# alibaba-damo-academy/Inferix

Hardware: AMD Instinct MI355X
Metric: latent_frames_per_sec (higher is better)
Workload: dtype bf16; 1 GPU; Self-Forcing 480p bf16 (Wan2.1-T2V-1.3B causal DiT, 30 layers), block_size=3, 21 latent frames = 7 blocks x (4 denoise + 1 context) generator forwards, KV prefix 4680..32760 keys in the KV manager's cache (identity page map; page-table form: `streaming_steady`); `value` counts the generator calls (SURVEY 8d), the per-block VAE decode of config 2 is measured beside it under --full (`per_block_decod; batch=1, parallelism=single, layers=30, pair_forwards=True, pair_mode=streams

## Files before the change

### inferix_amd/csrc/ifx_common.h

```cpp
#pragma once
#include <hip/hip_runtime.h>
#include <stdint.h>
#include <stdio.h>

#include "../../include/inferix_hip.h"

namespace ifx {

constexpr int kWave = 64;

typedef __attribute__((ext_vector_type(8))) __bf16 bf16x8;
typedef __attribute__((ext_vector_type(4))) __bf16 bf16x4;
typedef __attribute__((ext_vector_type(8))) unsigned short u16x8;
typedef __attribute__((ext_vector_type(4))) unsigned short u16x4;
typedef __attribute__((ext_vector_type(4))) short s16x4;
typedef __attribute__((ext_vector_type(4))) float f32x4;
typedef __attribute__((ext_vector_type(16))) float f32x16;
typedef __attribute__((ext_vector_type(4))) unsigned int u32x4;
typedef __attribute__((ext_vector_type(2))) unsigned int u32x2;

__device__ __forceinline__ float bf2f(unsigned short u) {
  return __builtin_bit_cast(float, (unsigned int)u << 16);
}
__device__ __forceinline__ unsigned short f2bf(float f) {
// ... 7 lines not shown
  float p = 0.17087277f;
  p = fmaf(p, t, -0.82215223f);
  p = fmaf(p, t, 1.48851587f);
  p = fmaf(p, t, -1.13520398f);
  p = fmaf(p, t, 0.27886807f);
  p = fmaf(p, t, -0.18628806f);
  p = fmaf(p, t, 0.09678418f);
  p = fmaf(p, t, 0.37409196f);
  p = fmaf(p, t, 1.00002368f);
  p = fmaf(p, t, -1.26551223f);
  const float arg = fmaf(-z, z, p);
  const float a = arg * 1.4426950408889634f;
  float r = fmaf(arg, 1.4426950408889634f, -a);
  r = fmaf(arg, 1.9259629911266175e-8f, r);
  const float ex = __builtin_amdgcn_exp2f(a) * fmaf(r, 0.6931471805599453f, 1.0f);
  const float erfc_z = t * ex;
  const float e = x >= 0.f ? 1.0f - erfc_z : erfc_z - 1.0f;
  return 0.5f * x * (1.0f + e);
}

__device__ __forceinline__ float gelu_tanh_fast(float x) {
  constexpr float c1 = -2.0f * 0.7978845608028654f * 1.4426950408889634f, c2 = c1 * 0.044715f;
  const float a = __builtin_fmaf(x * x, c2, c1) * x;
  return x * __builtin_amdgcn_rcpf(1.0f + __builtin_amdgcn_exp2f(a));
}

struct RowDivisor {
  float s, r;
  __device__ __forceinline__ explicit RowDivisor(float scale)
      : s(__builtin_bit_cast(float, __builtin_amdgcn_readfirstlane(__builtin_bit_cast(int, scale)))), r(__builtin_amdgcn_rcpf(s)) {}
  __device__ __forceinline__ bool fast() const { return s > 8.67361738e-19f && s < 1.15292150e18f; }
  template <bool FAST>
  __device__ __forceinline__ float div(float x) const {
    if (FAST) {
      const float q0 = x * r;
      const float e = __builtin_fmaf(-q0, s, x);
      return __builtin_fmaf(e, r, q0);
    }
    return x / s;
  }
};

template <int CTRL, int ROW_MASK>
__device__ __forceinline__ float dpp_or(float old, float v) {
  return __builtin_bit_cast(float, __builtin_amdgcn_update_dpp(__builtin_bit_cast(int, old), __builtin_bit_cast(int, v), CTRL, ROW_MASK, 0xf, false));
}
__device__ __forceinline__ float wave_sum(float v) {
  v += dpp_or<0xB1, 0xf>(0.f, v);
  v += dpp_or<0x4E, 0xf>(0.f, v);
  v += dpp_or<0x141, 0xf>(0.f, v);
  v += dpp_or<0x140, 0xf>(0.f, v);
  v += dpp_or<0x142, 0xa>(0.f, v);
  v += dpp_or<0x143, 0xc>(0.f, v);
  return __builtin_bit_cast(float, __builtin_amdgcn_readlane(__builtin_bit_cast(int, v), 63));
}
__device__ __forceinline__ float wave_max(float v) {
  v = fmaxf(v, dpp_or<0xB1, 0xf>(v, v));
  v = fmaxf(v, dpp_or<0x4E, 0xf>(v, v));
  v = fmaxf(v, dpp_or<0x141, 0xf>(v, v));
  v = fmaxf(v, dpp_or<0x140, 0xf>(v, v));
  v = fmaxf(v, dpp_or<0x142, 0xa>(v, v));
  v = fmaxf(v, dpp_or<0x143, 0xc>(v, v));
  return __builtin_bit_cast(float, __builtin_amdgcn_readlane(__builtin_bit_cast(int, v), 63));
}

struct KvAddr {
  const int32_t* pt;
  int32_t ps;
  int32_t seg_split, seg_delta;
  __device__ __forceinline__ int slot(int t) const {
    if (pt == nullptr) return (seg_split > 0 && t >= seg_split) ? t + seg_delta : t;
    int pg = t / ps;
    return pt[pg] * ps + (t - pg * ps);
  }
};

void set_error(const char* fmt, ...);
int check_launch(const char* what);
int gemm_variant();
int gemm_small_split();
unsigned* device_error_word();
long long spin_timeout_ticks();
int spin_fault();
int conv_variant();
unsigned* attn_debug_counter();
int attn_variant();

}

#define IFX_REQUIRE(cond, ...)            \
  do {                                    \
    if (!(cond)) {                        \
      ifx::set_error(__VA_ARGS__);        \
      return IFX_EINVAL;                  \
    }                                     \
  } while (0)
```

### inferix_amd/csrc/ifx_core.hip

```cpp
#include <stdarg.h>
#include <stdlib.h>
#include <string.h>

#include "ifx_common.h"

namespace ifx {
static thread_local char g_err[512] = "";

void set_error(const char* fmt, ...) {
  va_list ap;
  va_start(ap, fmt);
  vsnprintf(g_err, sizeof(g_err), fmt, ap);
  va_end(ap);
}

static int g_gemm_variant = -1, g_attn_variant = -1, g_conv_variant = -1, g_spin_timeout_ms = -1, g_spin_fault = 0;
static thread_local int g_gemm_small_split = -1;
static int opt_or_env(int& slot, const char* env, int dflt = 0) {
  if (slot < 0) {
    const char* e = getenv(env);
    slot = e ? atoi(e) : dflt;
  }
  return slot;
}
int gemm_variant() { return opt_or_env(g_gemm_variant, "IFX_GEMM_VARIANT"); }
int attn_variant() { return opt_or_env(g_attn_variant, "IFX_ATTN_VARIANT"); }
int conv_variant() { return opt_or_env(g_conv_variant, "IFX_CONV_VARIANT"); }
static unsigned* g_attn_dbg = nullptr;
static bool g_attn_dbg_on = false;
unsigned* attn_debug_counter() { return g_attn_dbg_on ? g_attn_dbg : nullptr; }
int gemm_small_split() { return opt_or_env(g_gemm_small_split, "IFX_GEMM_SMALL_SPLIT"); }

static unsigned* g_dev_err = nullptr;
unsigned* device_error_word() {
  if (g_dev_err == nullptr) {
    void* p = nullptr;
    if (hipHostMalloc(&p, 64, hipHostMallocMapped | hipHostMallocPortable) == hipSuccess && p != nullptr) {
      memset(p, 0, 64);
      g_dev_err = (unsigned*)p;
    }
  }
  return g_dev_err;
}
long long spin_timeout_ticks() { return (long long)max(1, opt_or_env(g_spin_timeout_ms, "IFX_SPIN_TIMEOUT_MS", 2000)) * 100000LL; }
int spin_fault() { return g_spin_fault; }
static thread_local char g_err_dev[640] = "";

int check_launch(const char* what) {
  hipError_t e = hipGetLastError();
  if (e != hipSuccess) {
    set_error("%s: launch failed: %s", what, hipGetErrorString(e));
    return IFX_ELAUNCH;
  }
  return IFX_OK;
}
}

extern "C" int ifx_version(void) { return (0 << 16) | (IFX_ABI_MINOR << 8) | 0; }
extern "C" int32_t ifx_device_error(int32_t clear) {
  unsigned* w = ifx::g_dev_err;
  if (w == nullptr) return 0;
  const unsigned v = __atomic_load_n(w, __ATOMIC_ACQUIRE);
  if (v != 0 && clear) __atomic_store_n(w, 0u, __ATOMIC_RELEASE);
  return (int32_t)v;
}
extern "C" const char* ifx_last_error(void) {
  const unsigned v = (unsigned)ifx_device_error(1);
  if (v == 0) return ifx::g_err;
  const unsigned kind = v >> 24, detail = v & 0xffffffu;
  snprintf(ifx::g_err_dev, sizeof(ifx::g_err_dev),
           "device: a kernel gave up a wait (%s, flag %u) after the spin budget — the producing workgroup was not resident or did not "
           "finish; the results of that launch are invalid%s%s",
           kind == 1 ? "split-K / stream-K consumer of ifx_gemm_bf16_ws / ifx_gemm_q8_ws" : "unknown waiter", detail,
           ifx::g_err[0] ? "; last host error: " : "", ifx::g_err);
  return ifx::g_err_dev;
}
extern "C" const char* ifx_arch(void) { return "gfx950"; }
extern "C" int ifx_set_option(const char* key, int32_t value) {
  if (key && !strcmp(key, "gemm_variant") && value >= 0 && value <= 29) { ifx::g_gemm_variant = value; return IFX_OK; }
  if (key && !strcmp(key, "gemm_small_split") && (value == 0 || value == 1)) { ifx::g_gemm_small_split = value; return IFX_OK; }
  if (key && !strcmp(key, "attn_variant") && value >= 0 && value <= 7) { ifx::g_attn_variant = value; return IFX_OK; }
  if (key && !strcmp(key, "conv_variant") && value >= 0 && value <= 1) { ifx::g_conv_variant = value; return IFX_OK; }
  if (key && !strcmp(key, "attn_debug_counters") && (value == 0 || value == 1)) {
    if (value == 1) {
      if (ifx::g_attn_dbg == nullptr && hipMalloc((void**)&ifx::g_attn_dbg, 64) != hipSuccess) {
        ifx::g_attn_dbg = nullptr;
        ifx::set_error("ifx_set_option: attn_debug_counters: hipMalloc failed");
        return IFX_ELAUNCH;
      }
      (void)hipDeviceSynchronize();
      (void)hipMemset(ifx::g_attn_dbg, 0, 64);
    }
    ifx::g_attn_dbg_on = value == 1;
    return IFX_OK;
  }
  if (key && !strcmp(key, "spin_timeout_ms") && value >= 1 && value <= 600000) { ifx::g_spin_timeout_ms = value; return IFX_OK; }
  if (key && !strcmp(key, "spin_fault") && (value == 0 || value == 1)) { ifx::g_spin_fault = value; return IFX_OK; }
  ifx::set_error("ifx_set_option: unknown key or value out of range: %s = %d", key ? key : "(null)", (int)value);
  return IFX_EINVAL;
}
extern "C" int ifx_get_option(const char* key, int32_t* value) {
  if (key == nullptr || value == nullptr) { ifx::set_error("ifx_get_option: null argument"); return IFX_EINVAL; }
  if (!strcmp(key, "gemm_variant")) { *value = ifx::gemm_variant(); return IFX_OK; }
  if (!strcmp(key, "gemm_small_split")) { *value = ifx::gemm_small_split(); return IFX_OK; }
  if (!strcmp(key, "attn_variant")) { *value = ifx::attn_variant(); return IFX_OK; }
  if (!strcmp(key, "conv_variant")) { *value = ifx::conv_variant(); return IFX_OK; }
  if (!strcmp(key, "attn_debug_counters")) { *value = ifx::g_attn_dbg_on ? 1 : 0; return IFX_OK; }
  if (!strcmp(key, "attn_rescale_count")) {
    unsigned v = 0;
    if (ifx::g_attn_dbg != nullptr) {
      (void)hipDeviceSynchronize();
      (void)hipMemcpy(&v, ifx::g_attn_dbg, sizeof(v), hipMemcpyDeviceToHost);
    }
    *value = (int32_t)(v & 0x7fffffffu);
    return IFX_OK;
  }
  if (!strcmp(key, "spin_timeout_ms")) { *value = (int32_t)(ifx::spin_timeout_ticks() / 100000LL); return IFX_OK; }
  if (!strcmp(key, "spin_fault")) { *value = ifx::spin_fault(); return IFX_OK; }
  ifx::set_error("ifx_get_option: unknown key: %s", key);
  return IFX_EINVAL;
}
```

### inferix_amd/csrc/ifx_gemm_pp.hip

```cpp
#include <stdlib.h>

#include <type_traits>

#include "ifx_common.h"

#ifndef IFX_PP_TRACE
#define IFX_PP_TRACE 0
#endif
#ifndef IFX_PP_LAB
#define IFX_PP_LAB IFX_PP_TRACE
#endif


namespace ifx {

struct EpiArgsP {
  const unsigned short* bias;
  const unsigned short* residual;
  int ld_res;
  const unsigned short* mod;
  int mod_slots, gate_slot, rows_per_group;
  const float* sa = nullptr;
  const float* sw = nullptr;
  const float* qdiv = nullptr;
  int q_via_bf16 = 0;
  unsigned short* y2 = nullptr;
  int ldy2 = 0, split_col = 0;
};

namespace gpp {
constexpr int BN = 256, BK = 64;
constexpr int SLOT = 16384, STAGE = 4 * SLOT, SCRATCH = 2 * STAGE;
constexpr int LDS_BYTES = SCRATCH + 32768;
constexpr int X_UP = 0, W_LO = SLOT, W_HI = 2 * SLOT, X_DN = 3 * SLOT;
typedef int v4i __attribute__((ext_vector_type(4)));
typedef int v8i __attribute__((ext_vector_type(8)));
typedef int v16i __attribute__((ext_vector_type(16)));
typedef __attribute__((address_space(3))) void* lds_ptr_t;

__device__ __forceinline__ void dma16(v4i rsrc, unsigned lds, int voff, int soff) {
  asm volatile("s_mov_b32 m0, %0\n\ts_nop 0\n\tbuffer_load_dwordx4 %1, %2, %3 offen lds"
               :
               : "s"(lds), "v"(voff), "s"(rsrc), "s"(soff)
               : "memory");
}
__device__ __forceinline__ v4i make_rsrc(const void* base, unsigned num_bytes) {
  const unsigned long long a = (unsigned long long)base;
  v4i r;
  r[0] = (int)(unsigned)a;
  r[1] = (int)((unsigned)(a >> 32) & 0xffffu);
  r[2] = (int)num_bytes;
  r[3] = 0x00020000;
  return r;
}
template <int N>
__device__ __forceinline__ void wait_vm() {
  asm volatile("s_waitcnt vmcnt(%0)" ::"n"(N) : "memory");
}
__device__ __forceinline__ void wait_lds() { __builtin_amdgcn_s_waitcnt(0xC07F); }

struct Cursor {
  int i, kt, g, rot, k0, len;
  int kb;
  unsigned stg;
  v4i rs;
};
}

template <int EPI, int TJ, int KS, int Q8 = 0>
__global__ __launch_bounds__(512, 2) void gemm_pp_kernel(const unsigned short* __restrict__ x, int ldx,
                                                         const unsigned short* __restrict__ w, unsigned short* __restrict__ y,
                                                         int ldy, int M, int N, int K, int tiles_m, int total, int per_xcd,
                                                         int wg_per_xcd, EpiArgsP ea, unsigned long long* __restrict__ trace, int dbg,
                                                         float* __restrict__ ws_part, unsigned* __restrict__ ws_flag,
                                                         unsigned* __restrict__ err_word, long long spin_ticks) {
  using namespace gpp;
  dbg = IFX_PP_LAB ? dbg : (dbg & 32);
  constexpr int BM = 64 * TJ;
  constexpr int GM = 4;
  constexpr bool RES = EPI == IFX_EPI_RESIDUAL || EPI == IFX_EPI_GATE_RES;
  extern __shared__ __attribute__((aligned(16))) unsigned char smem[];
  const int tid = threadIdx.x, lane = tid & 63;
  const int wave = __builtin_amdgcn_readfirstlane(tid >> 6);
  const int grp = wave >> 2, w4 = wave & 3;
  constexpr int ES = Q8 ? 1 : 2;
  const unsigned char* const xb = reinterpret_cast<const unsigned char*>(x);
  const unsigned char* const wb = reinterpret_cast<const unsigned char*>(w);
  constexpr bool SK = KS == 0;
  constexpr int KSD = KS > 0 ? KS : 1;
  const int S = K * ES / 128;
  const int KT = S / KSD;
  const int tiles_n = total / KSD / tiles_m;

  const int xcd = blockIdx.x & 7, slot_i = blockIdx.x >> 3;
  const int id_first = xcd * per_xcd + slot_i;
  const int id_end = min(xcd * per_xcd + per_xcd, total);
  if (!SK && id_first >= id_end) return;
  const int sk_P = (int)gridDim.x, sk_p = xcd * (sk_P >> 3) + slot_i;
  auto sk_start = [&](int q) __attribute__((always_inline)) { return (int)((long)q * total * S / sk_P); };
  const int sk_u0 = SK ? sk_start(sk_p) : 0, sk_u1 = SK ? sk_start(sk_p + 1) : 0;
  const int sk_t0 = SK ? sk_u0 / S : 0;
  const int n_my = SK ? (sk_u1 - 1) / S - sk_t0 + 1 : (id_end - id_first + wg_per_xcd - 1) / wg_per_xcd;
  const int G = SK ? sk_u1 - sk_u0 : n_my * KT;
  auto item_split = [&](int i) __attribute__((always_inline)) { return KS > 1 ? (id_first + i * wg_per_xcd) % KSD : 0; };
  auto item_tile = [&](int i) __attribute__((always_inline)) { return SK ? sk_t0 + i : (id_first + i * wg_per_xcd) / KSD; };
  auto item_k0 = [&](int i) __attribute__((always_inline)) { return SK ? (i == 0 ? sk_u0 - sk_t0 * S : 0) : item_split(i) * KT; };
  auto item_len = [&](int i) __attribute__((always_inline)) {
    return SK ? min(S, sk_u1 - (sk_t0 + i) * S) - (i == 0 ? sk_u0 - sk_t0 * S : 0) : KT;
  };
  auto item_dumps = [&](int i) __attribute__((always_inline)) { return SK ? (i == 0 && sk_u0 > sk_t0 * S) : (KS > 1 && item_split(i) >= 1); };
  auto item_parts = [&](int i) __attribute__((always_inline)) {
    if (!SK) return KS > 1 ? KS - 1 : 0;
    const int t_end = (sk_t0 + i + 1) * S;
    int n = 0;
    while (sk_p + 1 + n < sk_P && sk_start(sk_p + 1 + n) < t_end) ++n;
    return sk_u1 < t_end ? n : 0;
  };
  auto tile_base = [&](int i, int& m_base, int& n_base) __attribute__((always_inline)) {
    const int t_id = item_tile(i);
    const int grp_sz = GM * tiles_n;
    const int first_m = (t_id / grp_sz) * GM;
    const int gm = min(GM, tiles_m - first_m);
    const int rem = t_id % grp_sz;
    m_base = (first_m + rem % gm) * BM;
    n_base = (rem / gm) * BN;
  };

  const int r8 = lane >> 3, pc = lane & 7;
  const int prow = w4 * 8 + r8;
  const int ld_op = grp == 0 ? K : ldx;
  const int voff = prow * ld_op * ES + ((pc ^ ((prow >> 1) & 7)) << 4);
  const unsigned lds_piece0 = (unsigned)(unsigned long long)(lds_ptr_t)smem + w4 * 1024;
  auto cur_desc = [&](Cursor& c) __attribute__((always_inline)) {
    int mb, nb;
    tile_base(c.i, mb, nb);
    if (dbg & 1) mb = nb = 0;
    c.rot = (!SK && (dbg & 4)) ? ((nb / BN) * 3) % KT : 0;
    c.k0 = item_k0(c.i);
    c.len = item_len(c.i);
    c.kb = c.k0 * 128;
    if (grp == 0) c.rs = make_rsrc(wb + (size_t)nb * K * ES, (unsigned)min(((long)N - nb) * (long)K * ES, 0xffffffffL));
    else c.rs = make_rsrc(xb + (size_t)mb * ldx * ES, (unsigned)min(((long)M - mb - 1) * (long)ldx * ES + (long)K * ES, 0xffffffffL));
  };
  auto cur_init = [&](Cursor& c) __attribute__((always_inline)) {
    c.i = 0, c.kt = 0, c.g = 0, c.stg = 0;
    cur_desc(c);
  };
  auto cur_next = [&](Cursor& c) __attribute__((always_inline)) {
    ++c.g;
    c.stg ^= STAGE;
    c.kb += 128;
    if (++c.kt == c.len) {
      c.kt = 0;
      if (++c.i < n_my) cur_desc(c);
    }
  };
  auto issue = [&](const Cursor& c, int slot, int row0, int pieces) __attribute__((always_inline)) {
    const int kk = c.kt + c.rot;
    const int kb = IFX_PP_LAB ? ((!SK && kk >= KT ? kk - KT : kk) + c.k0) * 128 : c.kb;
    const unsigned p = lds_piece0 + c.stg + slot;
    if ((dbg & 8) && c.g >= 2) return;
#pragma unroll
    for (int q = 0; q < 4; ++q)
      if (q < pieces) dma16(c.rs, p + q * 4096, voff, kb + (row0 + q * 32) * ld_op * ES);
  };
  Cursor ca, cb;
  cur_init(ca);
  cur_init(cb);

  constexpr bool MF16 = Q8 == 0;
  const int l31 = lane & 31, hi = lane >> 5, l15 = lane & 15, q4 = lane >> 4;
  int lane_ks[4];
#pragma unroll
  for (int ks = 0; ks < 4; ++ks)
    lane_ks[ks] = MF16 ? l15 * 128 + ((((4 * ks + q4) & 7) ^ ((l15 >> 1) & 7)) << 4)
                       : l31 * 128 + (((2 * ks + hi) ^ ((l31 >> 1) & 7)) << 4);
  const int w_frag_off = (w4 >> 1) * SLOT + (w4 & 1) * 8192 + W_LO;
  const int x_frag_off = grp == 0 ? X_UP : X_DN;
  bf16x8 fx[4][TJ], fw[4][2], fx16[2 * TJ][2];
  int rg = 0;
  auto read_frags = [&]() __attribute__((always_inline)) {
    const unsigned char* st = smem + (rg & 1) * STAGE;
    if constexpr (MF16) {
#pragma unroll
      for (int kk = 0; kk < 2; ++kk) {
#pragma unroll
        for (int c = 0; c < 4; ++c) fw[c][kk] = *reinterpret_cast<const bf16x8*>(st + w_frag_off + lane_ks[kk] + c * 2048);
#pragma unroll
        for (int t = 0; t < 2 * TJ; ++t) fx16[t][kk] = *reinterpret_cast<const bf16x8*>(st + x_frag_off + lane_ks[kk] + t * 2048);
      }
    } else {
#pragma unroll
      for (int ks = 0; ks < 4; ++ks) {
#pragma unroll
        for (int i = 0; i < 2; ++i) fw[ks][i] = *reinterpret_cast<const bf16x8*>(st + w_frag_off + lane_ks[ks] + i * 4096);
#pragma unroll
        for (int j = 0; j < TJ; ++j) fx[ks][j] = *reinterpret_cast<const bf16x8*>(st + x_frag_off + lane_ks[ks] + j * 4096);
      }
    }
    ++rg;
  };

  f32x16 acc[2][TJ];
  f32x4 acc16[4][2 * TJ];
  auto quad = [&](int i, int j, int g) __attribute__((always_inline)) {
    if constexpr (MF16) return acc16[g][2 * j + i];
    else return f32x4{acc[i][j][4 * g], acc[i][j][4 * g + 1], acc[i][j][4 * g + 2], acc[i][j][4 * g + 3]};
  };
  auto mfma16 = [&](bool first) __attribute__((always_inline)) {
    const f32x4 z = {0.f, 0.f, 0.f, 0.f};
#pragma unroll
    for (int kk = 0; kk < 2; ++kk)
#pragma unroll
      for (int c = 0; c < 4; ++c)
#pragma unroll
        for (int t = 0; t < 2 * TJ; ++t)
          acc16[c][t] = __builtin_amdgcn_mfma_f32_16x16x32_bf16(fw[c][kk], fx16[t][kk], first && kk == 0 ? z : acc16[c][t], 0, 0, 0);
  };
  auto q8_mfma = [&](int kk, int i, int j, const f32x16 c) __attribute__((always_inline)) {
    const v8i a = __builtin_shufflevector(__builtin_bit_cast(v4i, fw[2 * kk][i]), __builtin_bit_cast(v4i, fw[2 * kk + 1][i]), 0, 1, 2, 3, 4, 5, 6, 7);
    const v8i b = __builtin_shufflevector(__builtin_bit_cast(v4i, fx[2 * kk][j]), __builtin_bit_cast(v4i, fx[2 * kk + 1][j]), 0, 1, 2, 3, 4, 5, 6, 7);
    return __builtin_amdgcn_mfma_scale_f32_32x32x64_f8f6f4(a, b, c, 0, 0, 0, 0x7f7f7f7f, 0, 0x7f7f7f7f);
  };
  auto i8_mfma = [&](int ks, int i, int j, const f32x16 c) __attribute__((always_inline)) {
    return __builtin_bit_cast(f32x16, __builtin_amdgcn_mfma_i32_32x32x32_i8(__builtin_bit_cast(v4i, fw[ks][i]), __builtin_bit_cast(v4i, fx[ks][j]),
                                                                            __builtin_bit_cast(v16i, c), 0, 0, 0));
  };
  auto mfma_first = [&]() __attribute__((always_inline)) {
    const f32x16 z = {0.f, 0.f, 0.f, 0.f, 0.f, 0.f, 0.f, 0.f, 0.f, 0.f, 0.f, 0.f, 0.f, 0.f, 0.f, 0.f};
    if constexpr (Q8 == 2) {
#pragma unroll
      for (int ks = 0; ks < 4; ++ks)
#pragma unroll
        for (int i = 0; i < 2; ++i)
#pragma unroll
          for (int j = 0; j < TJ; ++j) acc[i][j] = i8_mfma(ks, i, j, ks == 0 ? z : acc[i][j]);
      return;
    }
    if constexpr (Q8 == 1) {
#pragma unroll
      for (int i = 0; i < 2; ++i)
#pragma unroll
        for (int j = 0; j < TJ; ++j) acc[i][j] = q8_mfma(0, i, j, z);
#pragma unroll
      for (int i = 0; i < 2; ++i)
#pragma unroll
        for (int j = 0; j < TJ; ++j) acc[i][j] = q8_mfma(1, i, j, acc[i][j]);
      return;
    }
    mfma16(true);
  };
  auto mfma_next = [&]() __attribute__((always_inline)) {
    if constexpr (Q8 == 2) {
#pragma unroll
      for (int ks = 0; ks < 4; ++ks)
#pragma unroll
        for (int i = 0; i < 2; ++i)
#pragma unroll
          for (int j = 0; j < TJ; ++j) acc[i][j] = i8_mfma(ks, i, j, acc[i][j]);
      return;
    }
    if constexpr (Q8 == 1) {
#pragma unroll
      for (int kk = 0; kk < 2; ++kk)
#pragma unroll
        for (int i = 0; i < 2; ++i)
#pragma unroll
          for (int j = 0; j < TJ; ++j) acc[i][j] = q8_mfma(kk, i, j, acc[i][j]);
      return;
    }
    mfma16(false);
  };
// ... 219 lines not shown
      }
      wait_lds();
#pragma unroll
      for (int p = 0; p < 4; ++p) {
        const int mrow = p * 8 + rr;
        const int m = e_m0 + j * 32 + mrow;
        const u16x8 vv = *reinterpret_cast<const u16x8*>(rd + p * 1024 + ((cc ^ (mrow & 7)) << 4));
        if constexpr (RES) asm volatile("" : "+v"(e_res[j & 1][p]));
        if constexpr (EPI == IFX_EPI_GATE_RES) {
          if (j == 0 && p == 0) asm volatile("" : "+v"(e_gate[0]), "+v"(e_gate[1]));
        }
        u16x8 o;
        if constexpr (EPI == IFX_EPI_BIAS) {
          o = vv;
        } else if constexpr (EPI == IFX_EPI_GELU_TANH) {
          if (ea.gate_slot) {
#pragma unroll
            for (int e = 0; e < 8; ++e) o[e] = f2bf(gelu_erf_f(bf2f(vv[e])));
          } else {
#pragma unroll
            for (int e = 0; e < 8; ++e) o[e] = f2bf(gelu_tanh_fast(bf2f(vv[e])));
          }
        } else {
          const u16x8 rv = __builtin_bit_cast(u16x8, e_res[j & 1][p]);
          if constexpr (EPI == IFX_EPI_RESIDUAL) {
#pragma unroll
            for (int e = 0; e < 8; ++e) o[e] = f2bf(bf2f(rv[e]) + bf2f(vv[e]));
          } else {
            const u16x8 gv = __builtin_bit_cast(u16x8, m >= e_split ? e_gate[1] : e_gate[0]);
#pragma unroll
            for (int e = 0; e < 8; ++e) o[e] = f2bf(bf2f(rv[e]) + rbf(bf2f(vv[e]) * bf2f(gv[e])));
          }
        }
        if constexpr (Q8 && EPI == IFX_EPI_GELU_TANH) {
          if (ea.qdiv != nullptr) {
            unsigned wq[2];
#pragma unroll
            for (int h = 0; h < 2; ++h) {
              float t[4];
#pragma unroll
              for (int e = 0; e < 4; ++e) {
                const float q = fminf(fmaxf(bf2f(o[4 * h + e]) / e_qd[h][e], -448.0f), 448.0f);
                t[e] = ea.q_via_bf16 ? rbf(q) : q;
              }
              unsigned pk = __builtin_amdgcn_cvt_pk_fp8_f32(t[0], t[1], 0u, false);
              wq[h] = __builtin_amdgcn_cvt_pk_fp8_f32(t[2], t[3], pk, true);
            }
            if (m < M && n_ok)
              *reinterpret_cast<u32x2*>(reinterpret_cast<unsigned char*>(y) + (size_t)(e_m0 + rr + j * 32 + p * 8) * ldy + e_n0 + cc * 8) =
                  u32x2{wq[0], wq[1]};
            continue;
          }
        }
        if (m < M && n_ok) *reinterpret_cast<u16x8*>(yrow + (size_t)(j * 32 + p * 8) * ldo) = o;
      }
    }
  };

#if IFX_PP_TRACE
  unsigned long long seg[6] = {0, 0, 0, 0, 0, 0};
  unsigned long long t_last = __builtin_readcyclecounter();
  int seg_i = 0;
#define PP_STAMP()                                                 \
  do {                                                             \
    const unsigned long long t_now = __builtin_readcyclecounter(); \
    seg[seg_i] += t_now - t_last;                                  \
    t_last = t_now;                                                \
    seg_i = seg_i == 5 ? 0 : seg_i + 1;                            \
  } while (0)
#else
#define PP_STAMP() \
  do {             \
  } while (0)
#endif
#ifndef IFX_PP_STAGGER
#define IFX_PP_STAGGER 0
#endif
  auto roles = [&](auto stagger_tag) __attribute__((always_inline)) {
  constexpr bool reads_first = decltype(stagger_tag)::value;

  int kt = 0, it = 0;
  int klen = item_len(0);
  if (grp == 0) {
    issue(ca, W_LO, 0, 4), issue(ca, W_HI, 128, 4), cur_next(ca);
    wait_vm<0>();
    __builtin_amdgcn_s_barrier();
    for (int g = 0; g < G; ++g) {
      PP_STAMP();
      const bool epi = g > 0 && kt == 0;
      const bool issued = ca.g < G;
      const bool early_reads = reads_first && !epi;
      if (epi && KS != 1 && item_dumps(it - 1)) {
        if (issued) issue(ca, W_LO, 0, 4), issue(ca, W_HI, 128, 4), cur_next(ca);
        PP_STAMP();
        dump_partial(it - 1);
        wait_vm<0>();
        flag_pending = flag_of(it - 1) + 1;
        PP_STAMP();
        read_frags();
      } else if (epi) {
        if (KS != 1) consumer_sync(it - 1);
        epilogue(it - 1, [&]() __attribute__((always_inline)) {
          if (issued) issue(ca, W_LO, 0, 4), issue(ca, W_HI, 128, 4), cur_next(ca);
          PP_STAMP();
        });
        PP_STAMP();
        read_frags();
      } else if (early_reads) {
        read_frags();
        if (issued) issue(ca, W_LO, 0, 4), issue(ca, W_HI, 128, 4), cur_next(ca);
        PP_STAMP();
        PP_STAMP();
      } else {
        if (issued) issue(ca, W_LO, 0, 4), issue(ca, W_HI, 128, 4), cur_next(ca);
        PP_STAMP();
        PP_STAMP();
        read_frags();
      }
      wait_lds();
      __builtin_amdgcn_sched_barrier(0);
      PP_STAMP();
      __builtin_amdgcn_s_barrier();
      __builtin_amdgcn_sched_barrier(0);
      PP_STAMP();
      if (KS != 1 && flag_pending) {
        if (wave == 0 && !(dbg & 32)) __hip_atomic_store(ws_flag + flag_pending - 1, 1u, __ATOMIC_RELAXED, __HIP_MEMORY_SCOPE_AGENT);
        flag_pending = 0;
      }
      if (!(dbg & 2)) {
        if (kt == 0) mfma_first();
        else mfma_next();
      }
      if (++kt == klen) kt = 0, ++it, klen = it < n_my ? item_len(it) : 0;
      wait_vm<0>();
      __builtin_amdgcn_sched_barrier(0);
      PP_STAMP();
      __builtin_amdgcn_s_barrier();
      __builtin_amdgcn_sched_barrier(0);
    }
    if (KS != 1 && item_dumps(it - 1)) {
      dump_partial(it - 1);
      wait_vm<0>();
      flag_pending = flag_of(it - 1) + 1;
    } else {
      if (KS != 1) consumer_sync(it - 1);
      epilogue(it - 1, [&]() __attribute__((always_inline)) {});
    }
    if (KS != 1) {
      __builtin_amdgcn_s_barrier();
      if (flag_pending && wave == 0 && !(dbg & 32)) __hip_atomic_store(ws_flag + flag_pending - 1, 1u, __ATOMIC_RELAXED, __HIP_MEMORY_SCOPE_AGENT);
    }
  } else {
    issue(cb, X_UP, 0, TJ), cur_next(cb);
    issue(ca, X_DN, 32 * TJ, TJ), cur_next(ca);
    if (cb.g < G) issue(cb, X_UP, 0, TJ), cur_next(cb);
    if (G > 1) wait_vm<2 * TJ>();
    else wait_vm<TJ>();
    __builtin_amdgcn_s_barrier();
    if (G > 1) wait_vm<TJ>();
    else wait_vm<0>();
    __builtin_amdgcn_s_barrier();
    for (int g = 0; g < G; ++g) {
      PP_STAMP();
      const bool lower = ca.g < G, upper = cb.g < G;
      if (reads_first) {
        read_frags();
        if (lower) issue(ca, X_DN, 32 * TJ, TJ), cur_next(ca);
        if (upper) issue(cb, X_UP, 0, TJ), cur_next(cb);
        PP_STAMP();
        PP_STAMP();
      } else {
        if (lower) issue(ca, X_DN, 32 * TJ, TJ), cur_next(ca);
        if (upper) issue(cb, X_UP, 0, TJ), cur_next(cb);
        PP_STAMP();
        PP_STAMP();
        read_frags();
      }
      wait_lds();
      if (upper) wait_vm<2 * TJ>();
      else if (lower) wait_vm<TJ>();
      else wait_vm<0>();
      __builtin_amdgcn_sched_barrier(0);
      PP_STAMP();
      __builtin_amdgcn_s_barrier();
      __builtin_amdgcn_sched_barrier(0);
      PP_STAMP();
      if (!(dbg & 2)) {
        if (kt == 0) mfma_first();
        else mfma_next();
      }
      if (++kt == klen) kt = 0, ++it, klen = it < n_my ? item_len(it) : 0;
      if (upper) wait_vm<TJ>();
      else wait_vm<0>();
      __builtin_amdgcn_sched_barrier(0);
      PP_STAMP();
      if (kt == 0) {
        if (KS != 1 && item_dumps(it - 1)) {
          dump_partial(it - 1);
          wait_vm<0>();
        } else {
          if (KS != 1) consumer_sync(it - 1);
          epilogue(it - 1, [&]() __attribute__((always_inline)) {});
        }
      }
      if (g + 1 < G || KS != 1) {
        __builtin_amdgcn_s_barrier();
        __builtin_amdgcn_sched_barrier(0);
      }
    }
  }
  };
  if (IFX_PP_STAGGER && (w4 & 1)) roles(std::true_type{});
  else roles(std::false_type{});
#if IFX_PP_TRACE
  if (trace != nullptr && blockIdx.x == 0 && lane == 0 && (wave & 3) == 0) {
#pragma unroll
    for (int k = 0; k < 6; ++k) trace[grp * 8 + k] = seg[k];
    trace[grp * 8 + 6] = (unsigned long long)G;
  }
#endif
}

bool gemm_pp_split(int N, int K) {
  static int min_k = -1;
  if (min_k < 0) {
    const char* e = getenv("IFX_PP_SPLIT_MIN_K");
    min_k = e ? atoi(e) : 4096;
  }
  return K >= min_k && N <= 2048 && (K / 64) % 2 == 0;
}
size_t gemm_pp_stream_k_workspace_bytes() { return 4096 + (size_t)256 * 128 * 256 * 4; }
size_t gemm_pp_workspace_bytes(int M, int N, int K) {
  if (!gemm_pp_split(N, K)) return 0;
  const size_t tn = (size_t)(N + 255) / 256;
  const size_t t4 = (size_t)((M + 255) / 256) * tn, t3 = (size_t)((M + 191) / 192) * tn;
  if (t4 > 1024) return 0;
  const size_t b4 = t4 * 256 * 256 * 4, b3 = t3 <= 1024 ? t3 * 192 * 256 * 4 : 0;
  return 4096 + (b4 > b3 ? b4 : b3);
}

size_t gemm_pp_small_workspace_bytes(int M, int N, int ks) {
  if (ks <= 1) return 0;
  const size_t tiles = (size_t)((M + 127) / 128) * ((N + 255) / 256);
  return 4096 + tiles * (size_t)(ks - 1) * 128 * 256 * 4;
}

int launch_gemm_pp(const unsigned short* x, int ldx, const unsigned short* w, unsigned short* y, int ldy, int M, int N, int K,
                   int mode, const unsigned short* bias, const unsigned short* residual, int ld_res, const unsigned short* mod,
                   int mod_slots, int gate_slot, int rows_per_group, hipStream_t s, int tj, void* workspace, const float* q8_sa,
                   const float* q8_sw, const float* q8_qdiv, int q8_via_bf16, int stream_k, int q8_int8, int force_ks,
                   unsigned short* y2, int ldy2, int split_col) {
  using namespace gpp;
  const bool q8 = q8_sa != nullptr;
  EpiArgsP ea{bias, residual, ld_res, mod, mod_slots, gate_slot, rows_per_group, q8_sa, q8_sw, q8_qdiv, q8_via_bf16, y2, ldy2, split_col};
  if (y2 != nullptr && (q8 || split_col <= 0 || split_col % BN != 0 || split_col >= N || ldy2 % 8 != 0 || ((uintptr_t)y2 & 15))) {
    set_error("ifx_gemm_bf16: the second destination needs bf16 operands, 0 < split_col < N a multiple of %d, ldy2 %% 8 == 0 and a 16-byte aligned y2", BN);
    return IFX_EINVAL;
  }
  if (q8 && (K % 128 != 0 || ldx % 16 != 0 || ((uintptr_t)q8_sw & 15) || ((uintptr_t)q8_qdiv & 15))) {
    set_error("ifx_gemm_q8: the ping-pong tile needs K %% 128 == 0, ldx %% 16 == 0 and 16-byte aligned scale vectors (K = %d, ldx = %d)", K, ldx);
    return IFX_EINVAL;
  }
  if (N % 64 != 0 || K % 64 != 0) {
    set_error("ifx_gemm_bf16: the ping-pong tile needs N and K to be multiples of 64 (N = %d, K = %d)", N, K);
    return IFX_EINVAL;
  }
  if (mode == IFX_EPI_GATE_RES && rows_per_group < 32 * tj) {
    set_error("ifx_gemm_bf16: the ping-pong tile needs gate groups of at least %d rows (rows_per_group = %d)", 32 * tj, rows_per_group);
    return IFX_EINVAL;
  }
  const bool res = mode == IFX_EPI_RESIDUAL || mode == IFX_EPI_GATE_RES;
  if (((uintptr_t)bias & 7) || (res && (((uintptr_t)residual & 15) || ld_res % 8 != 0)) ||
      (mode == IFX_EPI_GATE_RES && ((uintptr_t)mod & 15))) {
    set_error("ifx_gemm_bf16: the ping-pong tile needs 8-byte aligned bias and 16-byte aligned residual / gate rows");
    return IFX_EINVAL;
  }
  static int cu_of_dev[16] = {0};
  int dev = 0, n_cu = 0;
  if (hipGetDevice(&dev) == hipSuccess && dev >= 0 && dev < 16) {
    if (cu_of_dev[dev] == 0) {
      int v = 0;
      cu_of_dev[dev] = hipDeviceGetAttribute(&v, hipDeviceAttributeMultiprocessorCount, dev) == hipSuccess && v > 0 ? v : 256;
    }
    n_cu = cu_of_dev[dev];
  }
  if (n_cu <= 0) n_cu = 256;
  const int BM = 64 * tj;
  const int tiles_m = (M + BM - 1) / BM, tiles_n = (N + BN - 1) / BN;
  int ks = stream_k ? 0 : ((tj == 4 || (tj == 3 && !q8)) && workspace != nullptr && gemm_pp_split(N, q8 ? K / 2 : K) &&
                           tiles_m * tiles_n <= 1024) ? 2 : 1;
  if (force_ks > 1) {
    if (q8 || stream_k || tj != 2 || workspace == nullptr || (K / 64) % force_ks != 0 || tiles_m * tiles_n * (force_ks - 1) > 1024 ||
        (force_ks != 2 && force_ks != 4 && force_ks != 8)) {
      set_error("ifx_gemm_bf16: the %d-way K split needs the bf16 128-token tile, a workspace, K / 64 divisible by it and at most 1024 partial slots",
                force_ks);
      return IFX_EINVAL;
    }
    ks = force_ks;
  }
  const int total = tiles_m * tiles_n * (ks ? ks : 1), per_xcd = (total + 7) / 8;
  int wg_per_xcd = min(per_xcd, max(1, n_cu / 8));
  if (stream_k) {
    const long units = (long)total * (K * (q8 ? 1 : 2) / 128);
    if (q8 || tj != 2 || workspace == nullptr || units < 8) {
      set_error("ifx_gemm_bf16: stream-K needs the bf16 128-token tile, a workspace and at least 8 K-steps");
      return IFX_EINVAL;
    }
    wg_per_xcd = (int)max(1L, min((long)min(n_cu, 256) / 8, units / 6 / 8));
  }
  const dim3 grid(wg_per_xcd * 8), block(512);
  unsigned* ws_flag = (unsigned*)workspace;
  float* ws_part = workspace ? (float*)((char*)workspace + 4096) : nullptr;
  static unsigned long long* trace = nullptr;
  static int dbg = -1;
  if (dbg < 0) {
    const char* e = getenv("IFX_PP_DEBUG");
    dbg = e ? atoi(e) : 0;
  }
  const int dbg_launch = dbg | (spin_fault() ? 32 : 0);
  unsigned* const err_word = device_error_word();
  const long long spin_ticks = spin_timeout_ticks();
#if IFX_PP_TRACE
  if (!trace) {
    const char* e = getenv("IFX_PP_TRACE_PTR");
    if (e) trace = (unsigned long long*)strtoull(e, nullptr, 0);
  }
#endif
#define IFX_LAUNCH_PP(E, T, S, Q)                                                                                                    \
  do {                                                                                                                               \
    static bool attr_set = false;                                                                                                    \
    if (!attr_set) {                                                                                                                 \
      (void)hipFuncSetAttribute((const void*)gemm_pp_kernel<E, T, S, Q>, hipFuncAttributeMaxDynamicSharedMemorySize, (int)LDS_BYTES); \
      attr_set = true;                                                                                                               \
    }                                                                                                                                \
    hipLaunchKernelGGL((gemm_pp_kernel<E, T, S, Q>), grid, block, LDS_BYTES, s, x, ldx, w, y, ldy, M, N, K, tiles_m, total, per_xcd, \
                       wg_per_xcd, ea, trace, dbg_launch, ws_part, ws_flag, err_word, spin_ticks);                                   \
  } while (0)
#define IFX_SWITCH_PP(T, S, Q)                                              \
  switch (mode) {                                                           \
    case IFX_EPI_BIAS: IFX_LAUNCH_PP(IFX_EPI_BIAS, T, S, Q); break;         \
    case IFX_EPI_GELU_TANH: IFX_LAUNCH_PP(IFX_EPI_GELU_TANH, T, S, Q); break; \
    case IFX_EPI_RESIDUAL: IFX_LAUNCH_PP(IFX_EPI_RESIDUAL, T, S, Q); break; \
    case IFX_EPI_GATE_RES: IFX_LAUNCH_PP(IFX_EPI_GATE_RES, T, S, Q); break; \
    default: set_error("ifx_gemm: the ping-pong tile has no epilogue %d", mode); return IFX_EINVAL; \
  }
  if (q8 && ks == 2) {
    if (q8_int8) { IFX_SWITCH_PP(4, 2, 2) }
    else { IFX_SWITCH_PP(4, 2, 1) }
  } else if (q8 && q8_int8) {
    if (tj == 4) { IFX_SWITCH_PP(4, 1, 2) }
    else if (tj == 3) { IFX_SWITCH_PP(3, 1, 2) }
    else if (tj == 2) { IFX_SWITCH_PP(2, 1, 2) }
    else { set_error("ifx_gemm_q8: no ping-pong tile of %d tokens", 64 * tj); return IFX_EINVAL; }
  } else if (q8) {
    if (tj == 4) { IFX_SWITCH_PP(4, 1, 1) }
    else if (tj == 3) { IFX_SWITCH_PP(3, 1, 1) }
    else if (tj == 2) { IFX_SWITCH_PP(2, 1, 1) }
    else { set_error("ifx_gemm_q8: no ping-pong tile of %d tokens", 64 * tj); return IFX_EINVAL; }
  } else if (ks == 0) {
    IFX_SWITCH_PP(2, 0, 0)
  } else if (tj == 2 && ks == 2) { IFX_SWITCH_PP(2, 2, 0)
  } else if (tj == 2 && ks == 4) { IFX_SWITCH_PP(2, 4, 0)
  } else if (tj == 2 && ks == 8) { IFX_SWITCH_PP(2, 8, 0)
  } else if (ks == 2) {
    if (tj == 4) { IFX_SWITCH_PP(4, 2, 0) }
    else { IFX_SWITCH_PP(3, 2, 0) }
  } else if (tj == 4) { IFX_SWITCH_PP(4, 1, 0) }
  else if (tj == 3) { IFX_SWITCH_PP(3, 1, 0) }
  else if (tj == 2) { IFX_SWITCH_PP(2, 1, 0) }
  else { set_error("ifx_gemm_bf16: no ping-pong tile of %d tokens", 64 * tj); return IFX_EINVAL; }
#undef IFX_SWITCH_PP
#undef IFX_LAUNCH_PP
  return check_launch("ifx_gemm_bf16(pp)");
}

}
```

Measured before the change: 21.62 frames/s.

## Add dedicated loader waves to the 128-token bf16 ping-pong GEMM tile

```diff
diff --git a/inferix_amd/csrc/ifx_common.h b/inferix_amd/csrc/ifx_common.h
--- a/inferix_amd/csrc/ifx_common.h
+++ b/inferix_amd/csrc/ifx_common.h
@@ -113,6 +113,7 @@
 unsigned* device_error_word();
 long long spin_timeout_ticks();
 int spin_fault();
+int gemm_pp_variant();
 int conv_variant();
 unsigned* attn_debug_counter();
 int attn_variant();
diff --git a/inferix_amd/csrc/ifx_core.hip b/inferix_amd/csrc/ifx_core.hip
--- a/inferix_amd/csrc/ifx_core.hip
+++ b/inferix_amd/csrc/ifx_core.hip
@@ -14,7 +14,7 @@
   va_end(ap);
 }
 
-static int g_gemm_variant = -1, g_attn_variant = -1, g_conv_variant = -1, g_spin_timeout_ms = -1, g_spin_fault = 0;
+static int g_gemm_variant = -1, g_gemm_pp_variant = -1, g_attn_variant = -1, g_conv_variant = -1, g_spin_timeout_ms = -1, g_spin_fault = 0;
 static thread_local int g_gemm_small_split = -1;
 static int opt_or_env(int& slot, const char* env, int dflt = 0) {
   if (slot < 0) {
@@ -24,6 +24,7 @@
   return slot;
 }
 int gemm_variant() { return opt_or_env(g_gemm_variant, "IFX_GEMM_VARIANT"); }
+int gemm_pp_variant() { return opt_or_env(g_gemm_pp_variant, "IFX_GEMM_PP_VARIANT"); }
 int attn_variant() { return opt_or_env(g_attn_variant, "IFX_ATTN_VARIANT"); }
 int conv_variant() { return opt_or_env(g_conv_variant, "IFX_CONV_VARIANT"); }
 static unsigned* g_attn_dbg = nullptr;
@@ -81,6 +82,7 @@
   if (key && !strcmp(key, "gemm_small_split") && (value == 0 || value == 1)) { ifx::g_gemm_small_split = value; return IFX_OK; }
   if (key && !strcmp(key, "attn_variant") && value >= 0 && value <= 7) { ifx::g_attn_variant = value; return IFX_OK; }
   if (key && !strcmp(key, "conv_variant") && value >= 0 && value <= 1) { ifx::g_conv_variant = value; return IFX_OK; }
+  if (key && !strcmp(key, "gemm_pp_variant") && value >= 0 && value <= 1) { ifx::g_gemm_pp_variant = value; return IFX_OK; }
   if (key && !strcmp(key, "attn_debug_counters") && (value == 0 || value == 1)) {
     if (value == 1) {
       if (ifx::g_attn_dbg == nullptr && hipMalloc((void**)&ifx::g_attn_dbg, 64) != hipSuccess) {
@@ -105,6 +107,7 @@
   if (!strcmp(key, "gemm_small_split")) { *value = ifx::gemm_small_split(); return IFX_OK; }
   if (!strcmp(key, "attn_variant")) { *value = ifx::attn_variant(); return IFX_OK; }
   if (!strcmp(key, "conv_variant")) { *value = ifx::conv_variant(); return IFX_OK; }
+  if (!strcmp(key, "gemm_pp_variant")) { *value = ifx::gemm_pp_variant(); return IFX_OK; }
   if (!strcmp(key, "attn_debug_counters")) { *value = ifx::g_attn_dbg_on ? 1 : 0; return IFX_OK; }
   if (!strcmp(key, "attn_rescale_count")) {
     unsigned v = 0;
diff --git a/inferix_amd/csrc/ifx_gemm_pp.hip b/inferix_amd/csrc/ifx_gemm_pp.hip
--- a/inferix_amd/csrc/ifx_gemm_pp.hip
+++ b/inferix_amd/csrc/ifx_gemm_pp.hip
@@ -33,6 +33,7 @@
 constexpr int SLOT = 16384, STAGE = 4 * SLOT, SCRATCH = 2 * STAGE;
 constexpr int LDS_BYTES = SCRATCH + 32768;
 constexpr int X_UP = 0, W_LO = SLOT, W_HI = 2 * SLOT, X_DN = 3 * SLOT;
+constexpr int LX_STAGE = 16384, LX_DN = 8192, LW_BASE = 32768, LW_STAGE = 32768;
 typedef int v4i __attribute__((ext_vector_type(4)));
 typedef int v8i __attribute__((ext_vector_type(8)));
 typedef int v16i __attribute__((ext_vector_type(16)));
@@ -57,6 +58,10 @@
 __device__ __forceinline__ void wait_vm() {
   asm volatile("s_waitcnt vmcnt(%0)" ::"n"(N) : "memory");
 }
+template <int N, bool ON>
+__device__ __forceinline__ void wait_vm_if() {
+  if constexpr (ON) wait_vm<N>();
+}
 __device__ __forceinline__ void wait_lds() { __builtin_amdgcn_s_waitcnt(0xC07F); }
 
 struct Cursor {
@@ -67,14 +72,15 @@
 };
 }
 
-template <int EPI, int TJ, int KS, int Q8 = 0>
-__global__ __launch_bounds__(512, 2) void gemm_pp_kernel(const unsigned short* __restrict__ x, int ldx,
+template <int EPI, int TJ, int KS, int Q8 = 0, int LW = 0>
+__global__ __launch_bounds__(LW ? 768 : 512, LW ? 3 : 2) void gemm_pp_kernel(const unsigned short* __restrict__ x, int ldx,
                                                          const unsigned short* __restrict__ w, unsigned short* __restrict__ y,
                                                          int ldy, int M, int N, int K, int tiles_m, int total, int per_xcd,
                                                          int wg_per_xcd, EpiArgsP ea, unsigned long long* __restrict__ trace, int dbg,
                                                          float* __restrict__ ws_part, unsigned* __restrict__ ws_flag,
                                                          unsigned* __restrict__ err_word, long long spin_ticks) {
   using namespace gpp;
+  static_assert(!LW || (TJ == 2 && KS == 1 && Q8 == 0), "the loader-wave form is the unsplit bf16 128-token tile");
   dbg = IFX_PP_LAB ? dbg : (dbg & 32);
   constexpr int BM = 64 * TJ;
   constexpr int GM = 4;
@@ -130,8 +136,10 @@
   const int prow = w4 * 8 + r8;
   const int ld_op = grp == 0 ? K : ldx;
   const int voff = prow * ld_op * ES + ((pc ^ ((prow >> 1) & 7)) << 4);
+  const int voff_w = LW ? prow * K * ES + ((pc ^ ((prow >> 1) & 7)) << 4) : 0;
+  const int voff_x = LW ? prow * ldx * ES + ((pc ^ ((prow >> 1) & 7)) << 4) : 0;
   const unsigned lds_piece0 = (unsigned)(unsigned long long)(lds_ptr_t)smem + w4 * 1024;
-  auto cur_desc = [&](Cursor& c) __attribute__((always_inline)) {
+  auto cur_desc = [&](Cursor& c, bool is_w) __attribute__((always_inline)) {
     int mb, nb;
     tile_base(c.i, mb, nb);
     if (dbg & 1) mb = nb = 0;
@@ -139,34 +147,44 @@
     c.k0 = item_k0(c.i);
     c.len = item_len(c.i);
     c.kb = c.k0 * 128;
-    if (grp == 0) c.rs = make_rsrc(wb + (size_t)nb * K * ES, (unsigned)min(((long)N - nb) * (long)K * ES, 0xffffffffL));
+    if (is_w) c.rs = make_rsrc(wb + (size_t)nb * K * ES, (unsigned)min(((long)N - nb) * (long)K * ES, 0xffffffffL));
     else c.rs = make_rsrc(xb + (size_t)mb * ldx * ES, (unsigned)min(((long)M - mb - 1) * (long)ldx * ES + (long)K * ES, 0xffffffffL));
   };
-  auto cur_init = [&](Cursor& c) __attribute__((always_inline)) {
+  auto cur_init = [&](Cursor& c, bool is_w) __attribute__((always_inline)) {
     c.i = 0, c.kt = 0, c.g = 0, c.stg = 0;
-    cur_desc(c);
-  };
-  auto cur_next = [&](Cursor& c) __attribute__((always_inline)) {
+    cur_desc(c, is_w);
+  };
+  auto cur_next = [&](Cursor& c, bool is_w) __attribute__((always_inline)) {
     ++c.g;
-    c.stg ^= STAGE;
+    if constexpr (LW) c.stg = !is_w ? c.stg ^ LX_STAGE : c.stg == 2 * LW_STAGE ? 0 : c.stg + LW_STAGE;
+    else c.stg ^= STAGE;
     c.kb += 128;
     if (++c.kt == c.len) {
       c.kt = 0;
-      if (++c.i < n_my) cur_desc(c);
-    }
-  };
-  auto issue = [&](const Cursor& c, int slot, int row0, int pieces) __attribute__((always_inline)) {
+      if (++c.i < n_my) cur_desc(c, is_w);
+    }
+  };
+  auto issue = [&](const Cursor& c, bool is_w, int slot, int row0, int pieces) __attribute__((always_inline)) {
     const int kk = c.kt + c.rot;
     const int kb = IFX_PP_LAB ? ((!SK && kk >= KT ? kk - KT : kk) + c.k0) * 128 : c.kb;
     const unsigned p = lds_piece0 + c.stg + slot;
     if ((dbg & 8) && c.g >= 2) return;
+    const int vo = LW ? (is_w ? voff_w : voff_x) : voff;
+    const int pitch = LW ? (is_w ? K : ldx) : ld_op;
 #pragma unroll
     for (int q = 0; q < 4; ++q)
-      if (q < pieces) dma16(c.rs, p + q * 4096, voff, kb + (row0 + q * 32) * ld_op * ES);
+      if (q < pieces) dma16(c.rs, p + q * 4096, vo, kb + (row0 + q * 32) * pitch * ES);
+  };
+  const bool opw = grp == 0;
+  auto req_w = [&](Cursor& c) __attribute__((always_inline)) {
+    if constexpr (!LW) issue(c, opw, W_LO, 0, 4), issue(c, opw, W_HI, 128, 4), cur_next(c, opw);
+  };
+  auto req_x = [&](Cursor& c, int slot, int row0) __attribute__((always_inline)) {
+    if constexpr (!LW) issue(c, opw, slot, row0, TJ), cur_next(c, opw);
   };
   Cursor ca, cb;
-  cur_init(ca);
-  cur_init(cb);
+  cur_init(ca, opw);
+  cur_init(cb, opw);
 
   constexpr bool MF16 = Q8 == 0;
   const int l31 = lane & 31, hi = lane >> 5, l15 = lane & 15, q4 = lane >> 4;
@@ -179,15 +197,20 @@
   const int x_frag_off = grp == 0 ? X_UP : X_DN;
   bf16x8 fx[4][TJ], fw[4][2], fx16[2 * TJ][2];
   int rg = 0;
+  int rw = 0;
+  const int w_off_lw = (w4 >> 1) * SLOT + (w4 & 1) * 8192, x_off_lw = grp == 0 ? 0 : LX_DN;
   auto read_frags = [&]() __attribute__((always_inline)) {
     const unsigned char* st = smem + (rg & 1) * STAGE;
+    const unsigned char* const wst = LW ? smem + LW_BASE + rw * LW_STAGE + w_off_lw : st + w_frag_off;
+    const unsigned char* const xst = LW ? smem + (rg & 1) * LX_STAGE + x_off_lw : st + x_frag_off;
+    if constexpr (LW) rw = rw == 2 ? 0 : rw + 1;
     if constexpr (MF16) {
 #pragma unroll
       for (int kk = 0; kk < 2; ++kk) {
 #pragma unroll
-        for (int c = 0; c < 4; ++c) fw[c][kk] = *reinterpret_cast<const bf16x8*>(st + w_frag_off + lane_ks[kk] + c * 2048);
-#pragma unroll
-        for (int t = 0; t < 2 * TJ; ++t) fx16[t][kk] = *reinterpret_cast<const bf16x8*>(st + x_frag_off + lane_ks[kk] + t * 2048);
+        for (int c = 0; c < 4; ++c) fw[c][kk] = *reinterpret_cast<const bf16x8*>(wst + lane_ks[kk] + c * 2048);
+#pragma unroll
+        for (int t = 0; t < 2 * TJ; ++t) fx16[t][kk] = *reinterpret_cast<const bf16x8*>(xst + lane_ks[kk] + t * 2048);
       }
     } else {
 #pragma unroll
@@ -573,8 +596,8 @@
   int kt = 0, it = 0;
   int klen = item_len(0);
   if (grp == 0) {
-    issue(ca, W_LO, 0, 4), issue(ca, W_HI, 128, 4), cur_next(ca);
-    wait_vm<0>();
+    req_w(ca);
+    wait_vm_if<0, !LW>();
     __builtin_amdgcn_s_barrier();
     for (int g = 0; g < G; ++g) {
       PP_STAMP();
@@ -582,7 +605,7 @@
       const bool issued = ca.g < G;
       const bool early_reads = reads_first && !epi;
       if (epi && KS != 1 && item_dumps(it - 1)) {
-        if (issued) issue(ca, W_LO, 0, 4), issue(ca, W_HI, 128, 4), cur_next(ca);
+        if (issued) req_w(ca);
         PP_STAMP();
         dump_partial(it - 1);
         wait_vm<0>();
@@ -592,18 +615,18 @@
       } else if (epi) {
         if (KS != 1) consumer_sync(it - 1);
         epilogue(it - 1, [&]() __attribute__((always_inline)) {
-          if (issued) issue(ca, W_LO, 0, 4), issue(ca, W_HI, 128, 4), cur_next(ca);
+          if (issued) req_w(ca);
           PP_STAMP();
         });
         PP_STAMP();
         read_frags();
       } else if (early_reads) {
         read_frags();
-        if (issued) issue(ca, W_LO, 0, 4), issue(ca, W_HI, 128, 4), cur_next(ca);
+        if (issued) req_w(ca);
         PP_STAMP();
         PP_STAMP();
       } else {
-        if (issued) issue(ca, W_LO, 0, 4), issue(ca, W_HI, 128, 4), cur_next(ca);
+        if (issued) req_w(ca);
         PP_STAMP();
         PP_STAMP();
         read_frags();
@@ -623,7 +646,7 @@
         else mfma_next();
       }
       if (++kt == klen) kt = 0, ++it, klen = it < n_my ? item_len(it) : 0;
-      wait_vm<0>();
+      wait_vm_if<0, !LW>();
       __builtin_amdgcn_sched_barrier(0);
       PP_STAMP();
       __builtin_amdgcn_s_barrier();
@@ -642,35 +665,35 @@
       if (flag_pending && wave == 0 && !(dbg & 32)) __hip_atomic_store(ws_flag + flag_pending - 1, 1u, __ATOMIC_RELAXED, __HIP_MEMORY_SCOPE_AGENT);
     }
   } else {
-    issue(cb, X_UP, 0, TJ), cur_next(cb);
-    issue(ca, X_DN, 32 * TJ, TJ), cur_next(ca);
-    if (cb.g < G) issue(cb, X_UP, 0, TJ), cur_next(cb);
-    if (G > 1) wait_vm<2 * TJ>();
-    else wait_vm<TJ>();
+    req_x(cb, X_UP, 0);
+    req_x(ca, X_DN, 32 * TJ);
+    if (cb.g < G) req_x(cb, X_UP, 0);
+    if (G > 1) wait_vm_if<2 * TJ, !LW>();
+    else wait_vm_if<TJ, !LW>();
     __builtin_amdgcn_s_barrier();
-    if (G > 1) wait_vm<TJ>();
-    else wait_vm<0>();
+    if (G > 1) wait_vm_if<TJ, !LW>();
+    else wait_vm_if<0, !LW>();
     __builtin_amdgcn_s_barrier();
     for (int g = 0; g < G; ++g) {
       PP_STAMP();
       const bool lower = ca.g < G, upper = cb.g < G;
       if (reads_first) {
         read_frags();
-        if (lower) issue(ca, X_DN, 32 * TJ, TJ), cur_next(ca);
-        if (upper) issue(cb, X_UP, 0, TJ), cur_next(cb);
+        if (lower) req_x(ca, X_DN, 32 * TJ);
+        if (upper) req_x(cb, X_UP, 0);
         PP_STAMP();
         PP_STAMP();
       } else {
-        if (lower) issue(ca, X_DN, 32 * TJ, TJ), cur_next(ca);
-        if (upper) issue(cb, X_UP, 0, TJ), cur_next(cb);
+        if (lower) req_x(ca, X_DN, 32 * TJ);
+        if (upper) req_x(cb, X_UP, 0);
         PP_STAMP();
         PP_STAMP();
         read_frags();
       }
       wait_lds();
-      if (upper) wait_vm<2 * TJ>();
-      else if (lower) wait_vm<TJ>();
-      else wait_vm<0>();
+      if (upper) wait_vm_if<2 * TJ, !LW>();
+      else if (lower) wait_vm_if<TJ, !LW>();
+      else wait_vm_if<0, !LW>();
       __builtin_amdgcn_sched_barrier(0);
       PP_STAMP();
       __builtin_amdgcn_s_barrier();
@@ -681,8 +704,8 @@
         else mfma_next();
       }
       if (++kt == klen) kt = 0, ++it, klen = it < n_my ? item_len(it) : 0;
-      if (upper) wait_vm<TJ>();
-      else wait_vm<0>();
+      if (upper) wait_vm_if<TJ, !LW>();
+      else wait_vm_if<0, !LW>();
       __builtin_amdgcn_sched_barrier(0);
       PP_STAMP();
       if (kt == 0) {
@@ -701,7 +724,51 @@
     }
   }
   };
-  if (IFX_PP_STAGGER && (w4 & 1)) roles(std::true_type{});
+  auto loader = [&]() __attribute__((always_inline)) {
+    Cursor cw, cu, cl;
+    cur_init(cw, true), cur_init(cu, false), cur_init(cl, false);
+    auto w_step = [&]() __attribute__((always_inline)) {
+      issue(cw, true, LW_BASE, 0, 4), issue(cw, true, LW_BASE + SLOT, 128, 4), cur_next(cw, true);
+    };
+    auto up_step = [&]() __attribute__((always_inline)) { issue(cu, false, 0, 0, TJ), cur_next(cu, false); };
+    auto lo_step = [&]() __attribute__((always_inline)) { issue(cl, false, LX_DN, 32 * TJ, TJ), cur_next(cl, false); };
+    w_step(), up_step();
+    if (G > 1) w_step();
+    lo_step();
+    if (G > 1) up_step(), wait_vm<8 + 2 * TJ>();
+    else wait_vm<TJ>();
+    __builtin_amdgcn_s_barrier();
+    __builtin_amdgcn_sched_barrier(0);
+#if IFX_PP_TRACE
+    t_last = __builtin_readcyclecounter();
+#endif
+    for (int g = 0; g < G; ++g) {
+      const bool more = g + 1 < G, more2 = g + 2 < G;
+      if (more2) w_step();
+      PP_STAMP();
+      if (more2) wait_vm<TJ + 8>();
+      else if (more) wait_vm<TJ>();
+      else wait_vm<0>();
+      __builtin_amdgcn_sched_barrier(0);
+      PP_STAMP();
+      __builtin_amdgcn_s_barrier();
+      __builtin_amdgcn_sched_barrier(0);
+      PP_STAMP();
+      if (more) lo_step();
+      if (more2) up_step();
+      PP_STAMP();
+      if (more2) wait_vm<8 + 2 * TJ>();
+      else if (more) wait_vm<TJ>();
+      else wait_vm<0>();
+      __builtin_amdgcn_sched_barrier(0);
+      PP_STAMP();
+      __builtin_amdgcn_s_barrier();
+      __builtin_amdgcn_sched_barrier(0);
+      PP_STAMP();
+    }
+  };
+  if (LW && grp == 2) loader();
+  else if (IFX_PP_STAGGER && (w4 & 1)) roles(std::true_type{});
   else roles(std::false_type{});
 #if IFX_PP_TRACE
   if (trace != nullptr && blockIdx.x == 0 && lane == 0 && (wave & 3) == 0) {
@@ -799,7 +866,7 @@
     }
     wg_per_xcd = (int)max(1L, min((long)min(n_cu, 256) / 8, units / 6 / 8));
   }
-  const dim3 grid(wg_per_xcd * 8), block(512);
+  const dim3 grid(wg_per_xcd * 8);
   unsigned* ws_flag = (unsigned*)workspace;
   float* ws_part = workspace ? (float*)((char*)workspace + 4096) : nullptr;
   static unsigned long long* trace = nullptr;
@@ -817,24 +884,25 @@
     if (e) trace = (unsigned long long*)strtoull(e, nullptr, 0);
   }
 #endif
-#define IFX_LAUNCH_PP(E, T, S, Q)                                                                                                    \
+#define IFX_LAUNCH_PP(E, T, S, Q, L)                                                                                                 \
   do {                                                                                                                               \
     static bool attr_set = false;                                                                                                    \
     if (!attr_set) {                                                                                                                 \
-      (void)hipFuncSetAttribute((const void*)gemm_pp_kernel<E, T, S, Q>, hipFuncAttributeMaxDynamicSharedMemorySize, (int)LDS_BYTES); \
+      (void)hipFuncSetAttribute((const void*)gemm_pp_kernel<E, T, S, Q, L>, hipFuncAttributeMaxDynamicSharedMemorySize, (int)LDS_BYTES); \
       attr_set = true;                                                                                                               \
     }                                                                                                                                \
-    hipLaunchKernelGGL((gemm_pp_kernel<E, T, S, Q>), grid, block, LDS_BYTES, s, x, ldx, w, y, ldy, M, N, K, tiles_m, total, per_xcd, \
-                       wg_per_xcd, ea, trace, dbg_launch, ws_part, ws_flag, err_word, spin_ticks);                                   \
+    hipLaunchKernelGGL((gemm_pp_kernel<E, T, S, Q, L>), grid, dim3(L ? 768 : 512), LDS_BYTES, s, x, ldx, w, y, ldy, M, N, K, tiles_m, \
+                       total, per_xcd, wg_per_xcd, ea, trace, dbg_launch, ws_part, ws_flag, err_word, spin_ticks);                   \
   } while (0)
-#define IFX_SWITCH_PP(T, S, Q)                                              \
-  switch (mode) {                                                           \
-    case IFX_EPI_BIAS: IFX_LAUNCH_PP(IFX_EPI_BIAS, T, S, Q); break;         \
-    case IFX_EPI_GELU_TANH: IFX_LAUNCH_PP(IFX_EPI_GELU_TANH, T, S, Q); break; \
-    case IFX_EPI_RESIDUAL: IFX_LAUNCH_PP(IFX_EPI_RESIDUAL, T, S, Q); break; \
-    case IFX_EPI_GATE_RES: IFX_LAUNCH_PP(IFX_EPI_GATE_RES, T, S, Q); break; \
+#define IFX_SWITCH_PP_L(T, S, Q, L)                                               \
+  switch (mode) {                                                                 \
+    case IFX_EPI_BIAS: IFX_LAUNCH_PP(IFX_EPI_BIAS, T, S, Q, L); break;            \
+    case IFX_EPI_GELU_TANH: IFX_LAUNCH_PP(IFX_EPI_GELU_TANH, T, S, Q, L); break;  \
+    case IFX_EPI_RESIDUAL: IFX_LAUNCH_PP(IFX_EPI_RESIDUAL, T, S, Q, L); break;    \
+    case IFX_EPI_GATE_RES: IFX_LAUNCH_PP(IFX_EPI_GATE_RES, T, S, Q, L); break;    \
     default: set_error("ifx_gemm: the ping-pong tile has no epilogue %d", mode); return IFX_EINVAL; \
   }
+#define IFX_SWITCH_PP(T, S, Q) IFX_SWITCH_PP_L(T, S, Q, 0)
   if (q8 && ks == 2) {
     if (q8_int8) { IFX_SWITCH_PP(4, 2, 2) }
     else { IFX_SWITCH_PP(4, 2, 1) }
@@ -858,9 +926,11 @@
     else { IFX_SWITCH_PP(3, 2, 0) }
   } else if (tj == 4) { IFX_SWITCH_PP(4, 1, 0) }
   else if (tj == 3) { IFX_SWITCH_PP(3, 1, 0) }
-  else if (tj == 2) { IFX_SWITCH_PP(2, 1, 0) }
+  else if (tj == 2 && gemm_pp_variant() == 1) { IFX_SWITCH_PP(2, 1, 0) }
+  else if (tj == 2) { IFX_SWITCH_PP_L(2, 1, 0, 1) }
   else { set_error("ifx_gemm_bf16: no ping-pong tile of %d tokens", 64 * tj); return IFX_EINVAL; }
 #undef IFX_SWITCH_PP
+#undef IFX_SWITCH_PP_L
 #undef IFX_LAUNCH_PP
   return check_launch("ifx_gemm_bf16(pp)");
 }
```

Result: faster. 22.00 frames/s (median of 6 runs) (+1.8%).
